# llm-d/llm-d-kv-cache-manager

Hardware: AMD Instinct MI355X
Metric: Score() QPS at 1M-block index, 64-pod fleet (higher is better)
Workload: dtype int64-hash/fp32-score; 1 GPU; model=meta-llama/Llama-3.1-8B-Instruct, global_batch=1048576, seq_len=8192, parallelism=single, index_blocks=1048576, num_pods=64, vocab=128256, block_size=16, keys_per_prompt=512, batch_per_call=32768

## Files before the change

### llmd_kvcache_amd/ops/csrc/hip_ops.hip

```cpp

#include <hip/hip_runtime.h>
#include <ATen/cuda/CUDAContext.h>

#include "kvidx_ops.h"

namespace kvidx {

#define DEV __device__ __forceinline__

DEV int64_t dev_table_find(const Table& v, uint64_t h, uint32_t model) {
  return probe_find(v.keys, v.meta, v.cap_mask, h, model);
}
DEV int64_t dev_emap_find(const Table& v, uint64_t h, uint32_t model) {
  return probe_find(v.e_keys, v.e_meta, v.cap_mask, h, model);
}

DEV int64_t dev_table_put(const Table& v, uint64_t h, uint32_t model,
                          int32_t epoch) {
  h = remap_hash(h);
  uint64_t s = probe_start(h, v.cap_mask);
  int64_t first_tomb = -1;
  int64_t victim = -1;
  int32_t victim_stamp = 0;
  for (int t = 0; t < PROBE_MAX; ++t) {
// ... 343 lines not shown
                               int64_t K, uint32_t model,
                               const uint64_t* __restrict__ filter,
                               int has_filter, int num_pods, int W,
                               int32_t epoch, int shard_id, int num_shards,
                               int n_tiers,
                               uint8_t* __restrict__ found,
                               unsigned long long* __restrict__ masks) {
  int64_t k = (int64_t)blockIdx.x * blockDim.x + threadIdx.x;
  if (k >= K) return;
  if (!owns_key(rh[k], shard_id, num_shards))
    return;
  found[k] = (uint8_t)dev_probe_collect(
      v, rh[k], model, filter, has_filter, num_pods, W, epoch,
      masks + (size_t)k * n_tiers * W, n_tiers);
}

DEV int score_walk_step(const unsigned long long* mk, int W, int n_tiers,
                        const float* __restrict__ weights, int lane,
                        bool first, int& active, float& score) {
  int cur = 0;
  float wmax = 0.f;
  for (int t = 0; t < n_tiers; ++t) {
    if ((mk[t * W] >> lane) & 1) {
      cur = 1;
      wmax = fmaxf(wmax, weights[t]);
    }
  }
  int act = first ? cur : (active & cur);
  active = act;
  if (act) score += wmax;
  return act;
}

DEV void fused_score_body(
    Table v, const uint64_t* __restrict__ h, const int K,
    uint32_t model, const uint64_t* __restrict__ filter, int has_filter,
    const float* __restrict__ weights, int num_pods, int W, int32_t epoch,
    int n_tiers, float* __restrict__ scores) {
  extern __shared__ unsigned long long lds_masks[];
  const int b = blockIdx.x;
  const int lane = threadIdx.x & 63;
  const int wave = threadIdx.x >> 6;

  for (int x = threadIdx.x; x < K * n_tiers * W; x += blockDim.x)
    lds_masks[x] = 0;
  __syncthreads();

  for (int k = threadIdx.x; k < K; k += blockDim.x)
    dev_probe_collect(v, h[k], model, filter, has_filter, num_pods, W, epoch,
                      lds_masks + (size_t)k * n_tiers * W, n_tiers);
  __syncthreads();

  for (int w = wave; w < W; w += 4) {
    float score = 0.f;
    int active = 0;
    for (int k = 0; k < K; ++k) {
      const int act =
          score_walk_step(lds_masks + (size_t)k * n_tiers * W + w, W, n_tiers,
                          weights, lane, k == 0, active, score);
      if (!__any(act)) break;
    }
    int pid = w * 64 + lane;
    if (pid < num_pods) scores[(size_t)b * num_pods + pid] = score;
  }
}

__global__ void __launch_bounds__(256) k_fused_score(
    Table v, const uint64_t* __restrict__ hashes,
    const int32_t* __restrict__ offsets,
    uint32_t model, const uint64_t* __restrict__ filter, int has_filter,
    const float* __restrict__ weights, int num_pods, int W, int32_t epoch,
    int n_tiers, float* __restrict__ scores) {
  const int b = blockIdx.x;
  fused_score_body(v, hashes + offsets[b], offsets[b + 1] - offsets[b], model,
                   filter, has_filter, weights, num_pods, W, epoch, n_tiers,
                   scores);
}

__global__ void __launch_bounds__(256) k_fused_score_rows(
    Table v, const uint64_t* __restrict__ hashes,
    const int32_t* __restrict__ n_keys,
    int64_t stride, uint32_t model, const uint64_t* __restrict__ filter,
    int has_filter, const float* __restrict__ weights, int num_pods, int W,
    int32_t epoch, int n_tiers, float* __restrict__ scores) {
  const int b = blockIdx.x;
  fused_score_body(v, hashes + (int64_t)b * stride, n_keys[b], model, filter,
                   has_filter, weights, num_pods, W, epoch, n_tiers, scores);
}

__global__ void __launch_bounds__(64) k_score_from_masks(
    const unsigned long long* __restrict__ masks,
    const int32_t* __restrict__ offsets,
    const float* __restrict__ weights, int T, int num_pods, int W,
    float* __restrict__ scores) {
  const int b = blockIdx.x;
  const int w_lo = blockIdx.y * 16;
  const int w_hi = min(W, w_lo + 16);
  const int WG = w_hi - w_lo;
  const int K = offsets[b + 1] - offsets[b];
  const int lane = threadIdx.x & 63;
  float score[16];
  int active[16];
  for (int w = 0; w < WG; ++w) {
    score[w] = 0.f;
    active[w] = 0;
  }
  for (int k = 0; k < K; ++k) {
    const unsigned long long* mk =
        masks + (size_t)(offsets[b] + k) * T * W;
    bool any = false;
    for (int w = 0; w < WG; ++w) {
      const int act = score_walk_step(mk + w_lo + w, W, T, weights, lane,
                                      k == 0, active[w], score[w]);
      if (__any(act)) any = true;
    }
    if (!any) break;
  }
  for (int w = 0; w < WG; ++w) {
    int pid = (w_lo + w) * 64 + lane;
    if (pid < num_pods) scores[(size_t)b * num_pods + pid] = score[w];
// ... 83 lines not shown
                          int64_t lane, int wl, int c, int max_chunks,
                          int64_t B) {
  const int cc = c & (CHAIN_STAGE_CHUNKS - 1);
  const int c0 = c - cc;
  const int n = cc + 1;
  const bool vec = (max_chunks & 1) == 0 &&
                   (reinterpret_cast<uintptr_t>(out) & 15) == 0;
  const int part2 = 2 * (wl & 7);
  __builtin_amdgcn_fence(__ATOMIC_RELEASE, "wavefront");
  __builtin_amdgcn_wave_barrier();
  __builtin_amdgcn_fence(__ATOMIC_ACQUIRE, "wavefront");
#pragma unroll
  for (int g = 0; g < 8; ++g) {
    const int r = g * 8 + (wl >> 3);
    const int64_t pb = lane - wl + r;
    const uint64_t* s = stage + r * CHAIN_STAGE_ROW + part2;
    const uint64_t v0 = s[0];
    const uint64_t v1 = s[1];
    if (pb < B && part2 < n) {
      uint64_t* o = out + pb * max_chunks + c0 + part2;
      if (vec) {
        *reinterpret_cast<u64x2*>(o) = u64x2{v0, v1};
      } else {
        o[0] = v0;
        if (part2 + 1 < n) o[1] = v1;
      }
    }
  }
  __builtin_amdgcn_fence(__ATOMIC_RELEASE, "wavefront");
  __builtin_amdgcn_wave_barrier();
  __builtin_amdgcn_fence(__ATOMIC_ACQUIRE, "wavefront");
}

template <int BS>
__global__ void k_fnv_chain_tr(const int32_t* __restrict__ tokens_t,
                               const uint64_t* __restrict__ parents,
                               const int32_t* __restrict__ n_chunks,
                               int64_t B, int max_chunks, int row_major,
                               uint64_t* __restrict__ out) {
  extern __shared__ uint64_t chain_stage[];
  const int64_t lane = (int64_t)blockIdx.x * blockDim.x + threadIdx.x;
  const int wl = threadIdx.x & 63;
  uint64_t* stage =
      chain_stage + (size_t)(threadIdx.x >> 6) * (64 * CHAIN_STAGE_ROW);
  const bool live = lane < B;
  const int64_t bi = live ? lane : 0;
  uint64_t h = parents[bi];
  const int mc = live ? n_chunks[bi] : 0;
  for (int c = 0; c < max_chunks; ++c) {
    uint32_t tok[BS];
#pragma unroll
    for (int j = 0; j < BS; ++j)
      tok[j] = (uint32_t)tokens_t[(int64_t)(c * BS + j) * B + bi];
    const bool active = c < mc;
    const bool wide = __all(!active || h > 0xFFFFFFFFull);
    const uint64_t h2 = chunk_hash_fast(h, tok, BS, wide);
    h = active ? h2 : h;
    const uint64_t val = active ? h : 0;
    const int cc = c & (CHAIN_STAGE_CHUNKS - 1);
    if (row_major)
      stage[wl * CHAIN_STAGE_ROW + cc] = val;
    else if (live)
      out[chain_out_index(row_major, lane, c, max_chunks, B)] = val;
    if (row_major && (cc == CHAIN_STAGE_CHUNKS - 1 || c == max_chunks - 1))
      chain_flush_rows(stage, out, lane, wl, c, max_chunks, B);
  }
}

template <int ALGO>
__global__ void k_apply_events(
    Table v, const int64_t* __restrict__ tokens,
    const int32_t* __restrict__ tok_off,
    const uint64_t* __restrict__ ehashes,
    const int32_t* __restrict__ eh_off,
    const uint64_t* __restrict__ parents,
    const uint8_t* __restrict__ has_parent,
    const uint8_t* __restrict__ ev_type,
    const uint32_t* __restrict__ pod_entry,
    const int32_t* __restrict__ grp_off,
    const int32_t* __restrict__ model_of,
    int64_t G, uint64_t init_hash, int block_size,
    int32_t epoch, int shard_id, int num_shards,
    uint64_t* __restrict__ req_scratch) {
  const int g = blockIdx.x * (blockDim.x >> 6) + (threadIdx.x >> 6);
  const int lane = threadIdx.x & 63;
  if (g >= G) return;
  const int e_begin = grp_off[g];
  const int e_end = grp_off[g + 1];

  for (int e = e_begin; e < e_end; ++e) {
    const int nh = eh_off[e + 1] - eh_off[e];
    const uint64_t* eh = ehashes + eh_off[e];
    const uint32_t model = (uint32_t)model_of[e];
    if (ev_type[e] == 1) {
      for (int i = lane; i < nh; i += 64)
        dev_remove_pods(v, eh[i], model, &pod_entry[e], 1);
      __builtin_amdgcn_wave_barrier();
      continue;
// ... 188 lines not shown
template <typename Kern, typename... Args>
static void launch_1d(Kern kernel, int64_t n, Args... args) {
  constexpr int threads = 256;
  hipLaunchKernelGGL(kernel, dim3((unsigned)((n + threads - 1) / threads)),
                     dim3(threads), 0, STREAM, args...);
}

static const uint64_t* filter_ptr(const at::Tensor& filter_words) {
  return filter_words.numel() > 0 ? u64p(filter_words) : nullptr;
}

static size_t fused_score_lds_bytes(int64_t max_k, int64_t n_tiers,
                                    int64_t W) {
  return (size_t)max_k * n_tiers * W * sizeof(uint64_t);
}
static bool fused_score_fits(int64_t max_k, int64_t n_tiers, int64_t W) {
  return W <= 16 && fused_score_lds_bytes(max_k, n_tiers, W) <= 64 * 1024;
}

template <typename Kern, typename... Where>
static at::Tensor launch_fused_score(Kern kernel, const Table& v, int64_t B,
                                     const at::Tensor& hashes,
                                     int64_t model_id,
                                     const at::Tensor& filter_words,
                                     const at::Tensor& weights,
                                     int64_t num_pods, int64_t epoch,
                                     int64_t max_k, int64_t n_tiers,
                                     Where... where) {
  int64_t W = pod_words(num_pods);
  TORCH_CHECK(W <= 16, "fused score supports up to 1024 pods");
  n_tiers = clamp_tiers(n_tiers);
  TORCH_CHECK(fused_score_fits(max_k, n_tiers, W),
              "fused score LDS overflow: reduce keys per prompt or pods");
  auto scores = at::zeros({B, num_pods}, hashes.options().dtype(at::kFloat));
  if (B == 0) return scores;
  const uint64_t* filter = filter_ptr(filter_words);
  hipLaunchKernelGGL(kernel, dim3((int)B), dim3(256),
                     fused_score_lds_bytes(max_k, n_tiers, W), STREAM, v,
                     (const uint64_t*)u64p(hashes), where...,
                     (uint32_t)model_id, filter, filter ? 1 : 0,
                     weights.data_ptr<float>(), (int)num_pods, (int)W,
                     (int32_t)epoch, (int)n_tiers, scores.data_ptr<float>());
  return scores;
}

template <typename F>
static void dispatch_chain_block_size(int64_t block_size, F&& f) {
  switch (block_size) {
    case 4:  f(std::integral_constant<int, 4>{});  break;
    case 8:  f(std::integral_constant<int, 8>{});  break;
    case 16: f(std::integral_constant<int, 16>{}); break;
    case 32: f(std::integral_constant<int, 32>{}); break;
    case 64: f(std::integral_constant<int, 64>{}); break;
    default:
      TORCH_CHECK(false, "hash_chain_tr supports block sizes 4/8/16/32/64; "
                         "use gpu_hash_chain for other sizes");
  }
}

struct RaggedPlan {
  int64_t B = 0, max_k = 0, total_chunks = 0;
  at::Tensor host;
};

static RaggedPlan plan_ragged(const at::Tensor& tokens,
                              const at::Tensor& offsets, int64_t block_size) {
  TORCH_CHECK(block_size > 0, "block_size must be positive");
  TORCH_CHECK(offsets.dtype() == at::kLong && offsets.dim() == 1 &&
                  offsets.numel() >= 1,
              "offsets must be an int64 [B+1] tensor");
  TORCH_CHECK(tokens.dim() == 1 &&
// ... 145 lines not shown
  launch_1d(k_get_request_keys, n, v, u64p(engine_hashes), n,
            (uint32_t)model_id, u8p(found), u64p(out));
  return {found, out};
}

std::vector<at::Tensor> kvidx::gpu_lookup(KVIDX_TABLE_PARAMS,
                                          at::Tensor request_hashes,
                                          int64_t model_id,
                                          at::Tensor filter_words,
                                          int64_t num_pods, int64_t epoch,
                                          int64_t shard_id, int64_t num_shards,
                                          int64_t n_tiers) {
  auto v = make_table_view(KVIDX_TABLE_ARGS, true);
  int64_t K = request_hashes.numel();
  int64_t W = pod_words(num_pods);
  n_tiers = clamp_tiers(n_tiers);
  auto found = at::zeros({K}, request_hashes.options().dtype(at::kByte));
  auto masks = at::zeros({K, n_tiers, W}, request_hashes.options());
  if (K == 0) return {found, masks};
  const uint64_t* filter = filter_ptr(filter_words);
  launch_1d(k_lookup_masks, K, v, u64p(request_hashes), K, (uint32_t)model_id,
            filter, filter ? 1 : 0, (int)num_pods, (int)W, (int32_t)epoch,
            (int)shard_id, (int)num_shards, (int)n_tiers, u8p(found),
            reinterpret_cast<unsigned long long*>(u64p(masks)));
  return {found, masks};
}

at::Tensor kvidx::gpu_fused_score(KVIDX_TABLE_PARAMS, at::Tensor hashes,
                                  at::Tensor offsets, int64_t model_id,
                                  at::Tensor filter_words, at::Tensor weights,
                                  int64_t num_pods, int64_t epoch,
                                  int64_t max_k, int64_t n_tiers) {
  auto v = make_table_view(KVIDX_TABLE_ARGS, true);
  return launch_fused_score(k_fused_score, v, offsets.numel() - 1, hashes,
                            model_id, filter_words, weights, num_pods, epoch,
                            max_k, n_tiers, (const int32_t*)i32p(offsets));
}

at::Tensor kvidx::gpu_fused_score_rows(KVIDX_TABLE_PARAMS, at::Tensor hashes,
                                       at::Tensor n_keys, int64_t model_id,
                                       at::Tensor filter_words,
                                       at::Tensor weights, int64_t num_pods,
                                       int64_t epoch, int64_t max_k,
                                       int64_t n_tiers) {
  auto v = make_table_view(KVIDX_TABLE_ARGS, true);
  TORCH_CHECK(hashes.is_cuda() && hashes.dtype() == at::kLong &&
                  hashes.dim() == 2 && hashes.is_contiguous(),
              "hashes must be a contiguous int64 [B, stride] device tensor");
  TORCH_CHECK(n_keys.is_cuda() && n_keys.dtype() == at::kInt &&
                  n_keys.is_contiguous(),
              "n_keys must be a contiguous int32 device tensor");
  int64_t B = hashes.size(0);
  int64_t stride = hashes.size(1);
  TORCH_CHECK(n_keys.numel() == B, "n_keys must have one entry per row");
  TORCH_CHECK(max_k <= stride, "max_k exceeds the row length");
  return launch_fused_score(k_fused_score_rows, v, B, hashes, model_id,
                            filter_words, weights, num_pods, epoch, max_k,
                            n_tiers, (const int32_t*)i32p(n_keys), stride);
}

at::Tensor kvidx::gpu_score_from_masks(at::Tensor masks, at::Tensor offsets,
                                       at::Tensor weights, int64_t num_pods) {
  int64_t B = offsets.numel() - 1;
  int64_t W = pod_words(num_pods);
  TORCH_CHECK(W <= 64, "score_from_masks supports up to 4096 pods");
  TORCH_CHECK(masks.dim() == 3, "masks must be [Ktot, T, W]");
  int64_t T = masks.size(1);
  auto scores = at::zeros({B, num_pods}, masks.options().dtype(at::kFloat));
  if (B == 0) return scores;
  int wgroups = (int)((W + 15) / 16);
  hipLaunchKernelGGL(
      k_score_from_masks, dim3((int)B, wgroups), dim3(64), 0, STREAM,
      reinterpret_cast<const unsigned long long*>(u64p(masks)),
      i32p(offsets), weights.data_ptr<float>(), (int)T, (int)num_pods, (int)W,
      scores.data_ptr<float>());
  return scores;
}

std::vector<at::Tensor> kvidx::gpu_hash_chain(
    at::Tensor tokens, at::Tensor tok_off, at::Tensor parents,
    int64_t block_size, int64_t algo) {
  TORCH_CHECK(tokens.is_cuda());
  TORCH_CHECK(algo_valid(algo), "unknown chain hash algo id ", algo);
  int64_t B = parents.numel();
  auto chunk_off_cpu = at::zeros({B + 1}, at::kLong);
  {
    auto off_cpu = tok_off.to(at::kCPU);
    const int64_t* offp = off_cpu.data_ptr<int64_t>();
    int64_t* cop = chunk_off_cpu.data_ptr<int64_t>();
    for (int64_t b = 0; b < B; ++b)
      cop[b + 1] = cop[b] + (offp[b + 1] - offp[b]) / block_size;
  }
  auto chunk_off = chunk_off_cpu.to(tokens.device());
  int64_t total = chunk_off_cpu.data_ptr<int64_t>()[B];
  auto out = at::empty({total}, tokens.options());
  if (B == 0) return {out, chunk_off};
  dispatch_algo(algo, [&](auto A) {
    launch_1d(k_hash_chain<decltype(A)::value>, B, tokens.data_ptr<int64_t>(),
              tok_off.data_ptr<int64_t>(), u64p(parents),
              chunk_off.data_ptr<int64_t>(), B, (int)block_size, u64p(out));
  });
  return {out, chunk_off};
}

at::Tensor kvidx::gpu_hash_chain_tr(at::Tensor tokens_t, at::Tensor parents,
                                    at::Tensor n_chunks, int64_t block_size,
                                    int64_t max_chunks, int64_t ilp,
                                    int64_t row_major, int64_t algo) {
  TORCH_CHECK(tokens_t.is_cuda() && tokens_t.dtype() == at::kInt);
  TORCH_CHECK(algo_valid(algo), "unknown chain hash algo id ", algo);
  TORCH_CHECK(ilp == 0 || ilp == 1,
              "gpu_hash_chain_tr runs one chain per lane: ilp must be 0 or 1 "
              "(the multi-chain and prefetch variants are gone), got ", ilp);
  TORCH_CHECK(tokens_t.dim() == 2, "tokens_t must be [T, B]");
  int64_t B = tokens_t.size(1);
  TORCH_CHECK(parents.numel() == B && n_chunks.numel() == B);
  auto out = at::empty(row_major ? std::initializer_list<int64_t>{B, max_chunks}
                                 : std::initializer_list<int64_t>{max_chunks, B},
                       parents.options());
  if (B == 0 || max_chunks == 0) return out;
  TORCH_CHECK(tokens_t.size(0) >= max_chunks * block_size,
              "tokens_t has fewer rows than max_chunks * block_size");
  auto tokens_c = tokens_t.contiguous();
  auto launch = [&](auto kern, int threads, size_t lds) {
    hipLaunchKernelGGL(kern, dim3((unsigned)((B + threads - 1) / threads)),
                       dim3(threads), lds, STREAM, i32p(tokens_c),
                       u64p(parents), i32p(n_chunks), B, (int)max_chunks,
                       (int)row_major, u64p(out));
  };
  dispatch_algo(algo, [&](auto A) {
    dispatch_chain_block_size(block_size, [&](auto S) {
      constexpr int AL = decltype(A)::value;
      constexpr int BS = decltype(S)::value;
      if constexpr (AL == ALGO_FNV64A)
        launch(k_fnv_chain_tr<BS>, 64, row_major ? chain_stage_bytes(64) : 0);
      else
        launch(k_sha_chain_tr<BS, AL>, sha_tr_threads(BS), 0);
    });
  });
  return out;
}

std::vector<at::Tensor> kvidx::gpu_stage_ragged_tokens(
    at::Tensor tokens, at::Tensor offsets, int64_t block_size) {
  auto p = plan_ragged(tokens, offsets, block_size);
  at::Device dev = tokens.is_cuda()
                       ? tokens.device()
                       : at::Device(at::kCUDA, at::cuda::current_device());
  return stage_ragged(p, tokens, block_size, dev);
}

at::Tensor kvidx::gpu_score_flat_tokens(KVIDX_TABLE_PARAMS,
                                        at::Tensor tokens_flat,
                                        at::Tensor offsets, int64_t model_id,
                                        at::Tensor filter_words,
                                        at::Tensor weights, int64_t num_pods,
                                        int64_t epoch, int64_t init_hash_bits,
                                        int64_t block_size, int64_t n_tiers,
                                        int64_t algo) {
  TORCH_CHECK(keys.is_cuda(), "table must live on the GPU");
  TORCH_CHECK(algo_valid(algo), "unknown chain hash algo id ", algo);
  auto p = plan_ragged(tokens_flat, offsets, block_size);
  auto dev = keys.device();
  auto fopt = at::TensorOptions().device(dev).dtype(at::kFloat);
  if (p.B == 0 || p.max_k == 0) return at::zeros({p.B, num_pods}, fopt);
  auto staged = stage_ragged(p, tokens_flat, block_size, dev);
  auto parents = at::full({p.B}, init_hash_bits, fopt.dtype(at::kLong));
  auto hashes = gpu_hash_chain_tr(staged[0], parents, staged[1], block_size,
                                  p.max_k, 0, 1, algo);
  if (fused_score_fits(p.max_k, clamp_tiers(n_tiers), pod_words(num_pods)))
// ... 131 lines not shown
```

### llmd_kvcache_amd/ops/csrc/bindings.cpp

```cpp

#include "kvidx_ops.h"

namespace kvidx::wire {
void register_wirefront(pybind11::module_& m);
}

PYBIND11_MODULE(TORCH_EXTENSION_NAME, m) {
  m.doc() = "MI355X-native KV-block index ops (CPU reference + gfx950 HIP)";
  m.def("tokens_to_chunk_hashes", &kvidx::tokens_to_chunk_hashes,
        py::arg("tokens"), py::arg("parent"), py::arg("block_size"),
        py::arg("algo") = 0);
  m.def("hash_chain_batch", &kvidx::hash_chain_batch,
        py::arg("tokens"), py::arg("offsets"), py::arg("parents"),
        py::arg("block_size"), py::arg("algo") = 0);
  m.def("tokens_to_chunk_hashes_fast", &kvidx::tokens_to_chunk_hashes_fast,
        py::arg("tokens"), py::arg("parent"), py::arg("block_size"),
        py::arg("algo") = 0);
  m.def("cpu_insert", &kvidx::cpu_insert);
  m.def("cpu_compact", &kvidx::cpu_compact);
  m.def("cpu_evict", &kvidx::cpu_evict);
  m.def("cpu_purge_pods", &kvidx::cpu_purge_pods);
  m.def("cpu_lookup", &kvidx::cpu_lookup);
  m.def("cpu_fused_score", &kvidx::cpu_fused_score);
  m.def("cpu_score_from_masks", &kvidx::cpu_score_from_masks);
  m.def("cpu_get_request_keys", &kvidx::cpu_get_request_keys);
#ifdef KVIDX_WITH_HIP
  m.attr("HAS_HIP") = true;
  m.def("gpu_insert", &kvidx::gpu_insert);
  m.def("gpu_compact", &kvidx::gpu_compact);
  m.def("gpu_evict", &kvidx::gpu_evict);
  m.def("gpu_purge_pods", &kvidx::gpu_purge_pods,
        py::call_guard<py::gil_scoped_release>());
  m.def("gpu_get_request_keys", &kvidx::gpu_get_request_keys);
  m.def("gpu_lookup", &kvidx::gpu_lookup);
  m.def("gpu_fused_score", &kvidx::gpu_fused_score);
  m.def("gpu_score_from_masks", &kvidx::gpu_score_from_masks);
  m.def("gpu_hash_chain", &kvidx::gpu_hash_chain,
        py::arg("tokens"), py::arg("tok_off"), py::arg("parents"),
        py::arg("block_size"), py::arg("algo") = 0);
  m.def("gpu_hash_chain_tr", &kvidx::gpu_hash_chain_tr,
        py::arg("tokens_t"), py::arg("parents"), py::arg("n_chunks"),
        py::arg("block_size"), py::arg("max_chunks"), py::arg("ilp") = 0,
        py::arg("row_major") = 0, py::arg("algo") = 0);
  m.def("gpu_fused_score_rows", &kvidx::gpu_fused_score_rows);
  m.def("gpu_stage_ragged_tokens", &kvidx::gpu_stage_ragged_tokens,
        py::arg("tokens"), py::arg("offsets"), py::arg("block_size"));
  m.def("gpu_score_flat_tokens", &kvidx::gpu_score_flat_tokens,
        py::arg("keys"), py::arg("meta"), py::arg("stamp"), py::arg("pods"),
        py::arg("e_keys"), py::arg("e_meta"), py::arg("e_vals"),
        py::arg("pods_per_key"), py::arg("tokens_flat"), py::arg("offsets"),
// ... 37 lines not shown
```

### llmd_kvcache_amd/ops/csrc/cpu_ops.cpp

```cpp

#include <cstring>

#include "kvidx_ops.h"

namespace kvidx {

static int64_t table_find(const Table& v, uint64_t h, uint32_t model) {
  return probe_find(v.keys, v.meta, v.cap_mask, h, model);
}
static int64_t emap_find(const Table& v, uint64_t h, uint32_t model) {
  return probe_find(v.e_keys, v.e_meta, v.cap_mask, h, model);
}

static int64_t table_put(const Table& v, uint64_t h, uint32_t model,
                         int32_t epoch) {
  h = remap_hash(h);
  uint64_t s = probe_start(h, v.cap_mask);
  int64_t first_tomb = -1;
  int64_t victim = -1;
  int32_t victim_stamp = 0;
  for (int t = 0; t < PROBE_MAX; ++t) {
    uint64_t i = (s + t) & v.cap_mask;
    uint64_t k = v.keys[i];
    uint32_t m = v.meta[i];
// ... 103 lines not shown
        h = chunk_hash_sha256(h, t, (int)block_size,
                              sha_digest_word(decltype(A)::value));
      out.push_back(h);
    }
  });
  return out;
}

std::vector<uint64_t> kvidx::tokens_to_chunk_hashes_fast(
    std::vector<uint64_t> tokens, uint64_t parent, int64_t block_size,
    int64_t algo) {
  TORCH_CHECK(block_size > 0, "block_size must be positive");
  std::vector<uint32_t> toks(tokens.begin(), tokens.end());
  int64_t n_chunks = (int64_t)toks.size() / block_size;
  std::vector<uint64_t> out;
  out.reserve(n_chunks);
  uint64_t h = parent;
  std::vector<uint32_t> words(
      16 * sha_blocks_for(sha_max_payload((int)block_size)));
  dispatch_algo(algo, [&](auto A) {
    for (int64_t c = 0; c < n_chunks; ++c) {
      const uint32_t* t = toks.data() + c * block_size;
      if constexpr (decltype(A)::value == ALGO_FNV64A) {
        h = chunk_hash_fast(h, t, (int)block_size, h > 0xFFFFFFFFull);
      } else {
        ShaHostBuf buf{words.data()};
        h = chunk_hash_sha256_wave(h, t, (int)block_size,
                                   sha_digest_word(decltype(A)::value), buf, true,
                                   ShaHostAny{});
      }
      out.push_back(h);
    }
  });
  return out;
}

std::vector<at::Tensor> kvidx::hash_chain_batch(
    at::Tensor tokens, at::Tensor offsets, at::Tensor parents,
    int64_t block_size, int64_t algo) {
  TORCH_CHECK(tokens.dtype() == at::kLong && offsets.dtype() == at::kLong &&
              parents.dtype() == at::kLong);
  TORCH_CHECK(block_size > 0, "block_size must be positive");
  auto tok = tokens.contiguous();
  auto off = offsets.contiguous();
  auto par = parents.contiguous();
  int64_t B = par.numel();
  const int64_t* offp = off.data_ptr<int64_t>();
  const int64_t* tokp = tok.data_ptr<int64_t>();
  const uint64_t* parp = u64p(par);

  auto chunk_off = at::zeros({B + 1}, tokens.options());
  int64_t* cop = chunk_off.data_ptr<int64_t>();
  for (int64_t b = 0; b < B; ++b)
    cop[b + 1] = cop[b] + (offp[b + 1] - offp[b]) / block_size;
  auto out = at::empty({cop[B]}, tokens.options());
  uint64_t* outp = u64p(out);

  dispatch_algo(algo, [&](auto A) {
    at::parallel_for(0, B, 1, [&](int64_t begin, int64_t end) {
      std::vector<uint32_t> buf(block_size);
      for (int64_t b = begin; b < end; ++b) {
        uint64_t h = parp[b];
        int64_t n_chunks = cop[b + 1] - cop[b];
        const int64_t* t0 = tokp + offp[b];
        for (int64_t c = 0; c < n_chunks; ++c) {
          for (int64_t j = 0; j < block_size; ++j)
// ... 289 lines not shown
```

### llmd_kvcache_amd/ops/csrc/kvidx_common.h

```cpp

#pragma once

#include <cstdint>

#ifdef KVIDX_DEBUG_ASSERTS
#if defined(__HIP_DEVICE_COMPILE__)
#define KVIDX_ASSERT(c) \
  do {                  \
    if (!(c)) __builtin_trap(); \
  } while (0)
#else
#include <cassert>
#define KVIDX_ASSERT(c) assert(c)
#endif
#else
#define KVIDX_ASSERT(c) ((void)0)
#endif

#if defined(__HIPCC__)
#define KVIDX_HD __host__ __device__ __forceinline__
#else
#define KVIDX_HD inline
#endif

// ... 85 lines not shown
  h = p1 ? h1 : h;
  return h;
}

KVIDX_HD uint64_t fnv_cbor_u64_branchless(uint64_t h, uint64_t v,
                                          uint8_t major) {
  const uint8_t mt = major << 5;
  const int sel = (v >= 24) + (v > 0xFF) + (v > 0xFFFF) +
                  (v > 0xFFFFFFFFull);
  const int n = sel == 0 ? 0 : (1 << (sel - 1));
  const uint8_t header = sel ? (uint8_t)(mt | (0x17 + sel))
                             : (uint8_t)(mt | v);
  h = fnv1a_64_byte(h, header);
#if defined(__HIP_DEVICE_COMPILE__)
#pragma unroll
#endif
  for (int k = 0; k < 8; ++k) {
    const uint8_t b = (uint8_t)(v >> (8 * (7 - k)));
    const uint64_t h2 = fnv1a_64_byte(h, b);
    h = (k >= 8 - n) ? h2 : h;
  }
  return h;
}

KVIDX_HD uint64_t fnv_cbor_u64_wide(uint64_t h, uint64_t v) {
  h = fnv1a_64_byte(h, 0x1B);
#if defined(__HIP_DEVICE_COMPILE__)
#pragma unroll
#endif
  for (int s = 56; s >= 0; s -= 8) h = fnv1a_64_byte(h, (uint8_t)(v >> s));
  return h;
}

template <typename TokT>
KVIDX_HD uint64_t chunk_hash_fast(uint64_t parent, const TokT* tokens,
                                  int n, bool wide_parent = false) {
  uint64_t h = FNV64_OFFSET;
  h = fnv1a_64_byte(h, 0x83);
  if (wide_parent)
    h = fnv_cbor_u64_wide(h, parent);
  else
    h = fnv_cbor_u64_branchless(h, parent, 0);
  h = fnv_cbor_u32_branchless(h, (uint32_t)n, 4);
#if defined(__HIP_DEVICE_COMPILE__)
#pragma unroll
#endif
  for (int i = 0; i < n; ++i)
    h = fnv_cbor_u32_branchless(h, (uint32_t)tokens[i], 0);
  h = fnv1a_64_byte(h, 0xF6);
  return h;
}

template <typename TokT>
KVIDX_HD uint64_t chunk_hash(uint64_t parent, const TokT* tokens, int n) {
  uint64_t h = FNV64_OFFSET;
  h = fnv1a_64_byte(h, 0x83);
  h = fnv_cbor_uint(h, parent, 0);
  h = fnv_cbor_uint(h, (uint64_t)n, 4);
  for (int i = 0; i < n; ++i) h = fnv_cbor_uint(h, (uint64_t)(uint32_t)tokens[i], 0);
  h = fnv1a_64_byte(h, 0xF6);
  return h;
}


static constexpr int ALGO_FNV64A = 0;
static constexpr int ALGO_SHA256_HI = 1;
static constexpr int ALGO_SHA256_LOW = 2;

KVIDX_HD bool algo_valid(int64_t algo) { return algo >= 0 && algo <= 2; }
KVIDX_HD constexpr int sha_digest_word(int algo) {
  return algo == ALGO_SHA256_LOW ? 6 : 0;
}

KVIDX_HD constexpr int sha_max_payload(int n) {
  return 1 + 9 + (n < 24 ? 1 : n <= 0xFF ? 2 : n <= 0xFFFF ? 3 : 5) + 5 * n +
         1;
}
KVIDX_HD constexpr int sha_blocks_for(int payload_bytes) {
  return (payload_bytes + 9 + 63) >> 6;
}

KVIDX_HD uint32_t sha_rotr(uint32_t x, int n) {
  return (x >> n) | (x << (32 - n));
// ... 310 lines not shown
```

### llmd_kvcache_amd/ops/csrc/kvidx_ops.h

```cpp

#pragma once

#include <torch/extension.h>

#include <type_traits>
#include <vector>

#include "kvidx_common.h"

#define KVIDX_TABLE_PARAMS                                                  \
  at::Tensor keys, at::Tensor meta, at::Tensor stamp, at::Tensor pods,      \
      at::Tensor e_keys, at::Tensor e_meta, at::Tensor e_vals,              \
      int64_t pods_per_key
#define KVIDX_TABLE_ARGS \
  keys, meta, stamp, pods, e_keys, e_meta, e_vals, pods_per_key

namespace kvidx {

std::vector<uint64_t> tokens_to_chunk_hashes(std::vector<uint64_t> tokens,
                                             uint64_t parent,
                                             int64_t block_size, int64_t algo);
std::vector<uint64_t> tokens_to_chunk_hashes_fast(std::vector<uint64_t> tokens,
                                                  uint64_t parent,
                                                  int64_t block_size,
                                                  int64_t algo);
std::vector<at::Tensor> hash_chain_batch(at::Tensor tokens, at::Tensor offsets,
                                         at::Tensor parents,
                                         int64_t block_size, int64_t algo);

void cpu_insert(KVIDX_TABLE_PARAMS, at::Tensor engine_hashes,
                at::Tensor request_hashes, int64_t model_id,
                at::Tensor pod_entries, int64_t epoch, int64_t shard_id,
                int64_t num_shards, int64_t emap_write);
void cpu_compact(KVIDX_TABLE_PARAMS, at::Tensor n_keys, at::Tensor n_meta,
                 at::Tensor n_stamp, at::Tensor n_pods, at::Tensor n_e_keys,
                 at::Tensor n_e_meta, at::Tensor n_e_vals);
void cpu_evict(KVIDX_TABLE_PARAMS, at::Tensor engine_hashes, int64_t model_id,
               at::Tensor pod_entries);
std::vector<int64_t> cpu_purge_pods(KVIDX_TABLE_PARAMS, at::Tensor purge_words,
                                    int64_t model_id);
std::vector<at::Tensor> cpu_lookup(KVIDX_TABLE_PARAMS,
                                   at::Tensor request_hashes, int64_t model_id,
                                   at::Tensor filter_words, int64_t num_pods,
                                   int64_t epoch, int64_t shard_id,
                                   int64_t num_shards, int64_t n_tiers);
at::Tensor cpu_fused_score(KVIDX_TABLE_PARAMS, at::Tensor hashes,
                           at::Tensor counts, int64_t model_id,
                           at::Tensor filter_words, at::Tensor weights,
                           int64_t num_pods, int64_t epoch);
at::Tensor cpu_score_from_masks(at::Tensor masks, at::Tensor offsets,
                                at::Tensor weights, int64_t num_pods);
std::vector<at::Tensor> cpu_get_request_keys(KVIDX_TABLE_PARAMS,
                                             at::Tensor engine_hashes,
                                             int64_t model_id);

#ifdef KVIDX_WITH_HIP
void gpu_insert(KVIDX_TABLE_PARAMS, at::Tensor engine_hashes,
                at::Tensor request_hashes, int64_t model_id,
// ... 129 lines not shown
```

Measured before the change: 33.86 million scores/s.

## Process fused-score keys in rounds with early exit on prefix break

The fused score kernel now probes keys in rounds of 256 (one key per thread), scores each round from LDS, and stops once any key in the round is missing or every pod's prefix chain has broken. This avoids probing the hash table for keys past the longest matching prefix, and LDS use is capped at one round instead of all keys. Each wave keeps per-pod-word scores in registers across rounds, and the output tensor is allocated with empty instead of zeros. The cost is extra block-wide barriers per round. Correctness depends on dev_probe_collect returning 1 when a key is found.

```diff
diff --git a/llmd_kvcache_amd/ops/csrc/hip_ops.hip b/llmd_kvcache_amd/ops/csrc/hip_ops.hip
--- a/llmd_kvcache_amd/ops/csrc/hip_ops.hip
+++ b/llmd_kvcache_amd/ops/csrc/hip_ops.hip
@@ -399,60 +399,100 @@
   return act;
 }
 
+constexpr int FUSED_SCORE_ROUND = 256;
+
+template <int R>
 DEV void fused_score_body(
     Table v, const uint64_t* __restrict__ h, const int K,
     uint32_t model, const uint64_t* __restrict__ filter, int has_filter,
     const float* __restrict__ weights, int num_pods, int W, int32_t epoch,
     int n_tiers, float* __restrict__ scores) {
   extern __shared__ unsigned long long lds_masks[];
+  constexpr int WAVES = R / 64;
+  constexpr int OWN = 16 / WAVES;
   const int b = blockIdx.x;
   const int lane = threadIdx.x & 63;
   const int wave = threadIdx.x >> 6;
-
-  for (int x = threadIdx.x; x < K * n_tiers * W; x += blockDim.x)
-    lds_masks[x] = 0;
-  __syncthreads();
-
-  for (int k = threadIdx.x; k < K; k += blockDim.x)
-    dev_probe_collect(v, h[k], model, filter, has_filter, num_pods, W, epoch,
-                      lds_masks + (size_t)k * n_tiers * W, n_tiers);
-  __syncthreads();
-
-  for (int w = wave; w < W; w += 4) {
-    float score = 0.f;
-    int active = 0;
-    for (int k = 0; k < K; ++k) {
-      const int act =
-          score_walk_step(lds_masks + (size_t)k * n_tiers * W + w, W, n_tiers,
-                          weights, lane, k == 0, active, score);
-      if (!__any(act)) break;
-    }
-    int pid = w * 64 + lane;
-    if (pid < num_pods) scores[(size_t)b * num_pods + pid] = score;
-  }
-}
-
-__global__ void __launch_bounds__(256) k_fused_score(
+  const int stride = n_tiers * W;
+
+  float score[OWN];
+  int active[OWN];
+  int live = 0;
+#pragma unroll
+  for (int i = 0; i < OWN; ++i) {
+    score[i] = 0.f;
+    active[i] = 0;
+    if (wave + i * WAVES < W) live |= 1 << i;
+  }
+
+  for (int k0 = 0; k0 < K; k0 += R) {
+    const int n = min(R, K - k0);
+    for (int x = threadIdx.x; x < n * stride; x += R) lds_masks[x] = 0;
+    __syncthreads();
+
+    int empty_key = 0;
+    if ((int)threadIdx.x < n) {
+      unsigned long long* mk = lds_masks + (size_t)threadIdx.x * stride;
+      const int found =
+          dev_probe_collect(v, h[k0 + threadIdx.x], model, filter, has_filter,
+                            num_pods, W, epoch, mk, n_tiers);
+      int any = 0;
+      if (found == 1)
+        for (int x = 0; x < stride; ++x) any |= mk[x] != 0;
+      empty_key = !any;
+    }
+    const bool last = __syncthreads_or(empty_key) || k0 + R >= K;
+
+#pragma unroll
+    for (int i = 0; i < OWN; ++i) {
+      if (!((live >> i) & 1)) continue;
+      const int w = wave + i * WAVES;
+      for (int k = 0; k < n; ++k) {
+        const int act =
+            score_walk_step(lds_masks + (size_t)k * stride + w, W, n_tiers,
+                            weights, lane, k0 + k == 0, active[i], score[i]);
+        if (!__any(act)) {
+          live &= ~(1 << i);
+          break;
+        }
+      }
+    }
+    if (last) break;
+    if (!__syncthreads_or(live)) break;
+  }
+
+#pragma unroll
+  for (int i = 0; i < OWN; ++i) {
+    const int pid = (wave + i * WAVES) * 64 + lane;
+    if (wave + i * WAVES < W && pid < num_pods)
+      scores[(size_t)b * num_pods + pid] = score[i];
+  }
+}
+
+template <int R>
+__global__ void __launch_bounds__(R) k_fused_score(
     Table v, const uint64_t* __restrict__ hashes,
     const int32_t* __restrict__ offsets,
     uint32_t model, const uint64_t* __restrict__ filter, int has_filter,
     const float* __restrict__ weights, int num_pods, int W, int32_t epoch,
     int n_tiers, float* __restrict__ scores) {
   const int b = blockIdx.x;
-  fused_score_body(v, hashes + offsets[b], offsets[b + 1] - offsets[b], model,
-                   filter, has_filter, weights, num_pods, W, epoch, n_tiers,
-                   scores);
-}
-
-__global__ void __launch_bounds__(256) k_fused_score_rows(
+  fused_score_body<R>(v, hashes + offsets[b], offsets[b + 1] - offsets[b],
+                      model, filter, has_filter, weights, num_pods, W, epoch,
+                      n_tiers, scores);
+}
+
+template <int R>
+__global__ void __launch_bounds__(R) k_fused_score_rows(
     Table v, const uint64_t* __restrict__ hashes,
     const int32_t* __restrict__ n_keys,
     int64_t stride, uint32_t model, const uint64_t* __restrict__ filter,
     int has_filter, const float* __restrict__ weights, int num_pods, int W,
     int32_t epoch, int n_tiers, float* __restrict__ scores) {
   const int b = blockIdx.x;
-  fused_score_body(v, hashes + (int64_t)b * stride, n_keys[b], model, filter,
-                   has_filter, weights, num_pods, W, epoch, n_tiers, scores);
+  fused_score_body<R>(v, hashes + (int64_t)b * stride, n_keys[b], model,
+                      filter, has_filter, weights, num_pods, W, epoch, n_tiers,
+                      scores);
 }
 
 __global__ void __launch_bounds__(64) k_score_from_masks(
@@ -888,11 +928,13 @@
   n_tiers = clamp_tiers(n_tiers);
   TORCH_CHECK(fused_score_fits(max_k, n_tiers, W),
               "fused score LDS overflow: reduce keys per prompt or pods");
-  auto scores = at::zeros({B, num_pods}, hashes.options().dtype(at::kFloat));
+  auto scores = at::empty({B, num_pods}, hashes.options().dtype(at::kFloat));
   if (B == 0) return scores;
   const uint64_t* filter = filter_ptr(filter_words);
-  hipLaunchKernelGGL(kernel, dim3((int)B), dim3(256),
-                     fused_score_lds_bytes(max_k, n_tiers, W), STREAM, v,
+  constexpr int64_t R = FUSED_SCORE_ROUND;
+  hipLaunchKernelGGL(kernel, dim3((int)B), dim3((int)R),
+                     fused_score_lds_bytes(std::min(max_k, R), n_tiers, W),
+                     STREAM, v,
                      (const uint64_t*)u64p(hashes), where...,
                      (uint32_t)model_id, filter, filter ? 1 : 0,
                      weights.data_ptr<float>(), (int)num_pods, (int)W,
@@ -1104,9 +1146,10 @@
                                   int64_t num_pods, int64_t epoch,
                                   int64_t max_k, int64_t n_tiers) {
   auto v = make_table_view(KVIDX_TABLE_ARGS, true);
-  return launch_fused_score(k_fused_score, v, offsets.numel() - 1, hashes,
-                            model_id, filter_words, weights, num_pods, epoch,
-                            max_k, n_tiers, (const int32_t*)i32p(offsets));
+  return launch_fused_score(k_fused_score<FUSED_SCORE_ROUND>, v,
+                            offsets.numel() - 1, hashes, model_id,
+                            filter_words, weights, num_pods, epoch, max_k,
+                            n_tiers, (const int32_t*)i32p(offsets));
 }
 
 at::Tensor kvidx::gpu_fused_score_rows(KVIDX_TABLE_PARAMS, at::Tensor hashes,
@@ -1126,9 +1169,10 @@
   int64_t stride = hashes.size(1);
   TORCH_CHECK(n_keys.numel() == B, "n_keys must have one entry per row");
   TORCH_CHECK(max_k <= stride, "max_k exceeds the row length");
-  return launch_fused_score(k_fused_score_rows, v, B, hashes, model_id,
-                            filter_words, weights, num_pods, epoch, max_k,
-                            n_tiers, (const int32_t*)i32p(n_keys), stride);
+  return launch_fused_score(k_fused_score_rows<FUSED_SCORE_ROUND>, v, B,
+                            hashes, model_id, filter_words, weights, num_pods,
+                            epoch, max_k, n_tiers,
+                            (const int32_t*)i32p(n_keys), stride);
 }
 
 at::Tensor kvidx::gpu_score_from_masks(at::Tensor masks, at::Tensor offsets,
```

Result: faster. 36.05 million scores/s (median of 6 runs) (+6.5%).

## Split FNV chain kernel into packer and hasher waves over double-buffered LDS

Applied to the files above, without the earlier changes.

The transposed FNV chain-hash kernel is restructured so that packer waves load tokens and encode each chunk into a packed CBOR byte stream in double-buffered LDS, while paired hasher waves consume that stream one dword at a time. A wave-wide max length bounds the loop. A gfx950 SDWA xor plus v_mad_u64_u32 sequence computes the per-byte FNV step, replacing per-token branchless CBOR hashing. The goal is to overlap global token loads and encoding with the serial hash chain and to cut per-byte ALU cost. In exchange the kernel gains a __syncthreads per chunk, extra LDS use, and inline assembly, and it only affects Score() to the extent that the chain hash sits on the scoring path.

```diff
diff --git a/llmd_kvcache_amd/ops/csrc/bindings.cpp b/llmd_kvcache_amd/ops/csrc/bindings.cpp
--- a/llmd_kvcache_amd/ops/csrc/bindings.cpp
+++ b/llmd_kvcache_amd/ops/csrc/bindings.cpp
@@ -16,6 +16,10 @@
   m.def("tokens_to_chunk_hashes_fast", &kvidx::tokens_to_chunk_hashes_fast,
         py::arg("tokens"), py::arg("parent"), py::arg("block_size"),
         py::arg("algo") = 0);
+  m.def("tokens_to_chunk_hashes_stream", &kvidx::tokens_to_chunk_hashes_stream,
+        py::arg("tokens"), py::arg("parent"), py::arg("block_size"));
+  m.def("chunk_stream_bytes", &kvidx::chunk_stream_bytes, py::arg("tokens"),
+        py::arg("block_size"), py::arg("reference") = false);
   m.def("cpu_insert", &kvidx::cpu_insert);
   m.def("cpu_compact", &kvidx::cpu_compact);
   m.def("cpu_evict", &kvidx::cpu_evict);
diff --git a/llmd_kvcache_amd/ops/csrc/cpu_ops.cpp b/llmd_kvcache_amd/ops/csrc/cpu_ops.cpp
--- a/llmd_kvcache_amd/ops/csrc/cpu_ops.cpp
+++ b/llmd_kvcache_amd/ops/csrc/cpu_ops.cpp
@@ -159,6 +159,49 @@
       out.push_back(h);
     }
   });
+  return out;
+}
+
+std::vector<uint64_t> kvidx::tokens_to_chunk_hashes_stream(
+    std::vector<uint64_t> tokens, uint64_t parent, int64_t block_size) {
+  TORCH_CHECK(block_size > 0 && block_size <= 256,
+              "block_size must be in (0, 256]");
+  std::vector<uint32_t> toks(tokens.begin(), tokens.end());
+  int64_t n_chunks = (int64_t)toks.size() / block_size;
+  std::vector<uint64_t> out;
+  out.reserve(n_chunks);
+  std::vector<uint8_t> buf(chunk_stream_max((int)block_size));
+  uint64_t h = parent;
+  for (int64_t c = 0; c < n_chunks; ++c) {
+    const int len = chunk_stream_encode(toks.data() + c * block_size,
+                                        (int)block_size, buf.data());
+    h = chunk_stream_hash(h, buf.data(), len, h > 0xFFFFFFFFull);
+    out.push_back(h);
+  }
+  return out;
+}
+
+std::vector<std::vector<uint8_t>> kvidx::chunk_stream_bytes(
+    std::vector<uint64_t> tokens, int64_t block_size, bool reference) {
+  TORCH_CHECK(block_size > 0 && block_size <= 256,
+              "block_size must be in (0, 256]");
+  std::vector<uint32_t> toks(tokens.begin(), tokens.end());
+  const int n = (int)block_size;
+  std::vector<std::vector<uint8_t>> out;
+  for (size_t c = 0; c + 1 <= toks.size() / (size_t)n; ++c) {
+    const uint32_t* t = toks.data() + c * n;
+    std::vector<uint8_t> buf(chunk_stream_max(n));
+    int len;
+    if (reference) {
+      len = cbor_put_uint(buf.data(), 0, (uint64_t)n, 4);
+      for (int i = 0; i < n; ++i) len = cbor_put_uint(buf.data(), len, t[i], 0);
+      buf[len++] = 0xF6;
+    } else {
+      len = chunk_stream_encode(t, n, buf.data());
+    }
+    buf.resize(len);
+    out.push_back(std::move(buf));
+  }
   return out;
 }
 
diff --git a/llmd_kvcache_amd/ops/csrc/hip_ops.hip b/llmd_kvcache_amd/ops/csrc/hip_ops.hip
--- a/llmd_kvcache_amd/ops/csrc/hip_ops.hip
+++ b/llmd_kvcache_amd/ops/csrc/hip_ops.hip
@@ -602,38 +602,108 @@
   __builtin_amdgcn_fence(__ATOMIC_ACQUIRE, "wavefront");
 }
 
+DEV uint32_t wave_max_u32(uint32_t v) {
+  auto fold = [](uint32_t a, uint32_t b) { return a > b ? a : b; };
+  v = fold(v, __builtin_amdgcn_update_dpp(v, v, 0xB1, 0xF, 0xF, false));
+  v = fold(v, __builtin_amdgcn_update_dpp(v, v, 0x4E, 0xF, 0xF, false));
+  v = fold(v, __builtin_amdgcn_update_dpp(v, v, 0x141, 0xF, 0xF, false));
+  v = fold(v, __builtin_amdgcn_update_dpp(v, v, 0x140, 0xF, 0xF, false));
+  return fold(fold(__builtin_amdgcn_readlane(v, 0), __builtin_amdgcn_readlane(v, 16)),
+              fold(__builtin_amdgcn_readlane(v, 32), __builtin_amdgcn_readlane(v, 48)));
+}
+
 template <int BS>
-__global__ void k_fnv_chain_tr(const int32_t* __restrict__ tokens_t,
-                               const uint64_t* __restrict__ parents,
-                               const int32_t* __restrict__ n_chunks,
-                               int64_t B, int max_chunks, int row_major,
-                               uint64_t* __restrict__ out) {
+struct ChainStreamLds {
+  static constexpr int NW = chunk_stream_words(BS);
+  uint32_t col[2][64 * NW];
+  uint32_t len[2][64];
+  uint32_t hi[2];
+};
+
+template <int BS, int PAIRS>
+__global__ void __launch_bounds__(128 * PAIRS) k_fnv_chain_tr(
+    const int32_t* __restrict__ tokens_t,
+    const uint64_t* __restrict__ parents,
+    const int32_t* __restrict__ n_chunks,
+    int64_t B, int max_chunks, int row_major,
+    uint64_t* __restrict__ out) {
   extern __shared__ uint64_t chain_stage[];
-  const int64_t lane = (int64_t)blockIdx.x * blockDim.x + threadIdx.x;
+  constexpr int NW = chunk_stream_words(BS);
+  constexpr int MINW = (chunk_stream_max(BS) - 4 * BS) >> 2;
+  __shared__ ChainStreamLds<BS> s_pairs[PAIRS];
   const int wl = threadIdx.x & 63;
-  uint64_t* stage =
-      chain_stage + (size_t)(threadIdx.x >> 6) * (64 * CHAIN_STAGE_ROW);
+  const int wave = __builtin_amdgcn_readfirstlane(threadIdx.x >> 6);
+  const bool packer = wave >= PAIRS;
+  const int pair = packer ? wave - PAIRS : wave;
+  ChainStreamLds<BS>& s = s_pairs[pair];
+  const int64_t lane = ((int64_t)blockIdx.x * PAIRS + pair) * 64 + wl;
   const bool live = lane < B;
   const int64_t bi = live ? lane : 0;
-  uint64_t h = parents[bi];
   const int mc = live ? n_chunks[bi] : 0;
-  for (int c = 0; c < max_chunks; ++c) {
+
+  if (packer) {
     uint32_t tok[BS];
+    auto load_chunk = [&](uint32_t* t, int c) {
+      const int cl = c < max_chunks ? c : max_chunks - 1;
+      const int32_t* p = tokens_t + (int64_t)cl * BS * B + bi;
 #pragma unroll
-    for (int j = 0; j < BS; ++j)
-      tok[j] = (uint32_t)tokens_t[(int64_t)(c * BS + j) * B + bi];
-    const bool active = c < mc;
-    const bool wide = __all(!active || h > 0xFFFFFFFFull);
-    const uint64_t h2 = chunk_hash_fast(h, tok, BS, wide);
-    h = active ? h2 : h;
-    const uint64_t val = active ? h : 0;
-    const int cc = c & (CHAIN_STAGE_CHUNKS - 1);
-    if (row_major)
-      stage[wl * CHAIN_STAGE_ROW + cc] = val;
-    else if (live)
-      out[chain_out_index(row_major, lane, c, max_chunks, B)] = val;
-    if (row_major && (cc == CHAIN_STAGE_CHUNKS - 1 || c == max_chunks - 1))
-      chain_flush_rows(stage, out, lane, wl, c, max_chunks, B);
+      for (int j = 0; j < BS; ++j, p += B) t[j] = (uint32_t)*p;
+    };
+    auto pack_chunk = [&](int c) {
+      uint32_t nxt[BS];
+      load_chunk(nxt, c + 1);
+      const int par = c & 1;
+      const uint32_t len = (uint32_t)chunk_stream_encode(
+          tok, BS, reinterpret_cast<uint8_t*>(s.col[par] + wl * NW));
+      s.len[par][wl] = len;
+      const bool counts = c < mc;
+      s.hi[par] = wave_max_u32(counts ? len : 0u);
+#pragma unroll
+      for (int j = 0; j < BS; ++j) tok[j] = nxt[j];
+    };
+    load_chunk(tok, 0);
+    pack_chunk(0);
+    __syncthreads();
+    for (int c = 0; c < max_chunks; ++c) {
+      if (c + 1 < max_chunks) pack_chunk(c + 1);
+      __syncthreads();
+    }
+  } else {
+    uint64_t* stage = chain_stage + (size_t)pair * (64 * CHAIN_STAGE_ROW);
+    uint64_t h = parents[bi];
+    __syncthreads();
+    for (int c = 0; c < max_chunks; ++c) {
+      const int par = c & 1;
+      const uint32_t* col = s.col[par] + wl * NW;
+      uint32_t d[NW];
+#pragma unroll
+      for (int i = 0; i < NW; ++i) d[i] = col[i];
+      const uint32_t len = s.len[par][wl];
+      const uint32_t vhi = s.hi[par];
+      const bool active = c < mc;
+      const bool wide = __all(!active || h > 0xFFFFFFFFull);
+      uint64_t g = chunk_hash_head(h, wide);
+      const int lw = (int)len >> 2;
+      const uint32_t part = col[lw];
+      const int nmax = (int)__builtin_amdgcn_readfirstlane(vhi) >> 2;
+#pragma unroll
+      for (int i = 0; i < NW; ++i) {
+        if (i >= MINW && i >= nmax) break;
+        const uint64_t g2 = fnv_stream_dword(g, d[i]);
+        g = (i < MINW || i < lw) ? g2 : g;
+      }
+      g = fnv_stream_tail(g, part, (int)len & 3);
+      h = active ? g : h;
+      const uint64_t val = active ? h : 0;
+      const int cc = c & (CHAIN_STAGE_CHUNKS - 1);
+      if (row_major)
+        stage[wl * CHAIN_STAGE_ROW + cc] = val;
+      else if (live)
+        out[chain_out_index(row_major, lane, c, max_chunks, B)] = val;
+      if (row_major && (cc == CHAIN_STAGE_CHUNKS - 1 || c == max_chunks - 1))
+        chain_flush_rows(stage, out, lane, wl, c, max_chunks, B);
+      __syncthreads();
+    }
   }
 }
 
@@ -1194,20 +1264,35 @@
   TORCH_CHECK(tokens_t.size(0) >= max_chunks * block_size,
               "tokens_t has fewer rows than max_chunks * block_size");
   auto tokens_c = tokens_t.contiguous();
-  auto launch = [&](auto kern, int threads, size_t lds) {
-    hipLaunchKernelGGL(kern, dim3((unsigned)((B + threads - 1) / threads)),
+  auto launch = [&](auto kern, int threads, int prompts, size_t lds) {
+    hipLaunchKernelGGL(kern, dim3((unsigned)((B + prompts - 1) / prompts)),
                        dim3(threads), lds, STREAM, i32p(tokens_c),
                        u64p(parents), i32p(n_chunks), B, (int)max_chunks,
                        (int)row_major, u64p(out));
   };
+  const bool two_pairs =
+      B > 64 * (int64_t)at::cuda::getCurrentDeviceProperties()
+                   ->multiProcessorCount;
   dispatch_algo(algo, [&](auto A) {
     dispatch_chain_block_size(block_size, [&](auto S) {
       constexpr int AL = decltype(A)::value;
       constexpr int BS = decltype(S)::value;
-      if constexpr (AL == ALGO_FNV64A)
-        launch(k_fnv_chain_tr<BS>, 64, row_major ? chain_stage_bytes(64) : 0);
-      else
-        launch(k_sha_chain_tr<BS, AL>, sha_tr_threads(BS), 0);
+      if constexpr (AL == ALGO_FNV64A) {
+        constexpr bool fits2 = sizeof(ChainStreamLds<BS>) * 2 +
+                                   chain_stage_bytes(128) <= 64 * 1024;
+        if constexpr (fits2) {
+          if (two_pairs) {
+            launch(k_fnv_chain_tr<BS, 2>, 256, 128,
+                   row_major ? chain_stage_bytes(128) : 0);
+            return;
+          }
+        }
+        launch(k_fnv_chain_tr<BS, 1>, 128, 64,
+               row_major ? chain_stage_bytes(64) : 0);
+      } else {
+        launch(k_sha_chain_tr<BS, AL>, sha_tr_threads(BS), sha_tr_threads(BS),
+               0);
+      }
     });
   });
   return out;
diff --git a/llmd_kvcache_amd/ops/csrc/kvidx_common.h b/llmd_kvcache_amd/ops/csrc/kvidx_common.h
--- a/llmd_kvcache_amd/ops/csrc/kvidx_common.h
+++ b/llmd_kvcache_amd/ops/csrc/kvidx_common.h
@@ -141,15 +141,20 @@
   return h;
 }
 
-template <typename TokT>
-KVIDX_HD uint64_t chunk_hash_fast(uint64_t parent, const TokT* tokens,
-                                  int n, bool wide_parent = false) {
+KVIDX_HD uint64_t chunk_hash_head(uint64_t parent, bool wide_parent) {
   uint64_t h = FNV64_OFFSET;
   h = fnv1a_64_byte(h, 0x83);
   if (wide_parent)
     h = fnv_cbor_u64_wide(h, parent);
   else
     h = fnv_cbor_u64_branchless(h, parent, 0);
+  return h;
+}
+
+template <typename TokT>
+KVIDX_HD uint64_t chunk_hash_fast(uint64_t parent, const TokT* tokens,
+                                  int n, bool wide_parent = false) {
+  uint64_t h = chunk_hash_head(parent, wide_parent);
   h = fnv_cbor_u32_branchless(h, (uint32_t)n, 4);
 #if defined(__HIP_DEVICE_COMPILE__)
 #pragma unroll
@@ -158,6 +163,102 @@
     h = fnv_cbor_u32_branchless(h, (uint32_t)tokens[i], 0);
   h = fnv1a_64_byte(h, 0xF6);
   return h;
+}
+
+
+KVIDX_HD constexpr int chunk_stream_max(int n) {
+  return (n < 24 ? 1 : n <= 0xFF ? 2 : n <= 0xFFFF ? 3 : 5) + 5 * n + 1;
+}
+KVIDX_HD constexpr int chunk_stream_words(int n) {
+  return ((chunk_stream_max(n) + 3) >> 2) | 1;
+}
+
+KVIDX_HD int chunk_stream_put_u32(uint8_t* p, uint32_t v) {
+  const bool p1 = v >= 24, p2 = v > 0xFF, p4 = v > 0xFFFF;
+  const int nv = (int)p1 + (int)p2 + 2 * (int)p4;
+  const uint8_t info = p4 ? 26 : p2 ? 25 : p1 ? 24 : (uint8_t)v;
+  const uint32_t x = v << ((32 - 8 * nv) & 31);
+  p[0] = info;
+#if defined(__HIP_DEVICE_COMPILE__)
+  const uint32_t y = __builtin_bswap32(x);
+  __builtin_memcpy(p + 1, &y, 4);
+#else
+  p[1] = (uint8_t)(x >> 24);
+  p[2] = (uint8_t)(x >> 16);
+  p[3] = (uint8_t)(x >> 8);
+  p[4] = (uint8_t)x;
+#endif
+  return 1 + nv;
+}
+
+template <typename TokT>
+KVIDX_HD int chunk_stream_encode(const TokT* tokens, int n, uint8_t* buf) {
+  int len = cbor_put_uint(buf, 0, (uint64_t)n, 4);
+#if defined(__HIP_DEVICE_COMPILE__)
+#pragma unroll
+#endif
+  for (int i = 0; i < n; ++i)
+    len += chunk_stream_put_u32(buf + len, (uint32_t)tokens[i]);
+  buf[len++] = 0xF6;
+  return len;
+}
+
+#if defined(__HIP_DEVICE_COMPILE__) && defined(__gfx950__)
+#define KVIDX_XOR_SEL(SEL)                                                  \
+  asm("v_xor_b32_sdwa %0, %1, %2 dst_sel:DWORD dst_unused:UNUSED_PAD "     \
+      "src0_sel:DWORD src1_sel:" SEL : "=v"(lo) : "v"((uint32_t)h), "v"(d))
+template <int K>
+__device__ __forceinline__ uint64_t fnv1a_64_byte_of(uint64_t h, uint32_t d) {
+  static_assert(FNV64_PRIME == ((1ull << 40) | 0x1B3ull), "split below");
+  uint32_t lo;
+  if constexpr (K == 0) KVIDX_XOR_SEL("BYTE_0");
+  else if constexpr (K == 1) KVIDX_XOR_SEL("BYTE_1");
+  else if constexpr (K == 2) KVIDX_XOR_SEL("BYTE_2");
+  else KVIDX_XOR_SEL("BYTE_3");
+  const uint32_t t = (uint32_t)(h >> 32) * 0x1B3u + (lo << 8);
+  const uint64_t pair = ((uint64_t)t << 32) | lo;
+  uint64_t out, carry;
+  asm("v_mad_u64_u32 %0, %1, %2, %3, %4"
+      : "=v"(out), "=s"(carry)
+      : "v"(lo), "s"(0x1B2u), "v"(pair));
+  return out;
+}
+#undef KVIDX_XOR_SEL
+#else
+template <int K>
+KVIDX_HD uint64_t fnv1a_64_byte_of(uint64_t h, uint32_t d) {
+  return fnv1a_64_byte(h, (uint8_t)(d >> (8 * K)));
+}
+#endif
+
+KVIDX_HD uint64_t fnv_stream_dword(uint64_t h, uint32_t d) {
+  h = fnv1a_64_byte_of<0>(h, d);
+  h = fnv1a_64_byte_of<1>(h, d);
+  h = fnv1a_64_byte_of<2>(h, d);
+  h = fnv1a_64_byte_of<3>(h, d);
+  return h;
+}
+KVIDX_HD uint64_t fnv_stream_tail(uint64_t h, uint32_t d, int r) {
+  const uint64_t h0 = fnv1a_64_byte_of<0>(h, d);
+  h = 0 < r ? h0 : h;
+  const uint64_t h1 = fnv1a_64_byte_of<1>(h, d);
+  h = 1 < r ? h1 : h;
+  const uint64_t h2 = fnv1a_64_byte_of<2>(h, d);
+  h = 2 < r ? h2 : h;
+  return h;
+}
+
+KVIDX_HD uint64_t chunk_stream_hash(uint64_t parent, const uint8_t* stream,
+                                    int len, bool wide_parent = false) {
+  uint64_t h = chunk_hash_head(parent, wide_parent);
+  auto dword = [&](int w) {
+    uint32_t d = 0;
+    for (int k = 0; k < 4 && 4 * w + k < len; ++k)
+      d |= (uint32_t)stream[4 * w + k] << (8 * k);
+    return d;
+  };
+  for (int w = 0; w < (len >> 2); ++w) h = fnv_stream_dword(h, dword(w));
+  return fnv_stream_tail(h, dword(len >> 2), len & 3);
 }
 
 template <typename TokT>
diff --git a/llmd_kvcache_amd/ops/csrc/kvidx_ops.h b/llmd_kvcache_amd/ops/csrc/kvidx_ops.h
--- a/llmd_kvcache_amd/ops/csrc/kvidx_ops.h
+++ b/llmd_kvcache_amd/ops/csrc/kvidx_ops.h
@@ -24,6 +24,10 @@
                                                   uint64_t parent,
                                                   int64_t block_size,
                                                   int64_t algo);
+std::vector<uint64_t> tokens_to_chunk_hashes_stream(
+    std::vector<uint64_t> tokens, uint64_t parent, int64_t block_size);
+std::vector<std::vector<uint8_t>> chunk_stream_bytes(
+    std::vector<uint64_t> tokens, int64_t block_size, bool reference);
 std::vector<at::Tensor> hash_chain_batch(at::Tensor tokens, at::Tensor offsets,
                                          at::Tensor parents,
                                          int64_t block_size, int64_t algo);
```

Measured after the change: 34.12 million scores/s before, 36.14 million scores/s after, median of 6. 5.9% higher.
